# gkirgizov/die

Measured on AMD Instinct MI355X. Metric: env steps/sec on 4096^2 Physarum grid, higher is better.
Workload: dtype f32

## Files before the change

die_amd/csrc/die_pic.hip:

```cpp
#include "die_forward.h"
#include <stdlib.h>

typedef uint32_t pic_u4v __attribute__((ext_vector_type(4)));
typedef uint32_t pic_u2v __attribute__((ext_vector_type(2)));
template <typename T> struct Vec4;
template <> struct Vec4<float> {
    static __device__ __forceinline__ void ld(const float* p, float v[4]) {
        const uint4 t = *(const uint4*)p;
        v[0] = __uint_as_float(t.x); v[1] = __uint_as_float(t.y); v[2] = __uint_as_float(t.z); v[3] = __uint_as_float(t.w);
    }
    static __device__ __forceinline__ void st(float* p, const float v[4]) {
        *(uint4*)p = make_uint4(__float_as_uint(v[0]), __float_as_uint(v[1]), __float_as_uint(v[2]), __float_as_uint(v[3]));
    }
    static __device__ __forceinline__ void st_sel(bool nt, float* p, const float v[4]) {
        if (!nt) { st(p, v); return; }
        pic_u4v t; t.x = __float_as_uint(v[0]); t.y = __float_as_uint(v[1]); t.z = __float_as_uint(v[2]); t.w = __float_as_uint(v[3]);
        __builtin_nontemporal_store(t, (pic_u4v*)p);
    }
};
template <> struct Vec4<__half> {
    static __device__ __forceinline__ void ld(const __half* p, float v[4]) {
        const uint2 t = *(const uint2*)p;
        const __half2 a = *(const __half2*)&t.x, b = *(const __half2*)&t.y;
        v[0] = __low2float(a); v[1] = __high2float(a); v[2] = __low2float(b); v[3] = __high2float(b);
// ... 23 lines not shown
    uint32_t *off, *n, *s, *inc;
};

struct PicArgs {
    die_geo g;
    int ntx, nty, xs, ys;
    uint32_t xcd_wb_mul;
    int rp_c, rp_f;
    int margin;
    int fm_r, fm_c;
    uint32_t mg_c, mg_f;
    PicLayout in, out;
    float* dep;
    float *adx, *ady, *adep;
    const void* food;
    float rate_feed, w_dep, w_dist;
    int boundary, cost;
    long long* part_gain;
    uint32_t* error;
    uint4* rim;
    uint8_t* rim_code;
    uint32_t* rim_cnt;
    int rim_cap, rim_r;
    int sub_mode, sub_tx0, sub_ty0, sub_ntx, sub_nty;
    int halo_fresh;
    const float *ipgx, *ipgy;
    float *opgx, *opgy;
    const uint16_t* order;
    int order_len;
};
__device__ __forceinline__ void pic_xcd_tile(int& tx, int& ty, int ntx, uint32_t row0, uint32_t wb_mul, uint32_t nty) {
    const uint32_t wb = nty >> 3, banded = (wb << 3) * (uint32_t)ntx;
    const uint32_t L = (blockIdx.y - row0) * nty + blockIdx.x;
    if (wb == 0) return;
    if (L < banded) {
        const uint32_t k = L >> 3;
        tx = (int)(wb_mul ? __umulhi(k, wb_mul) : k / wb); ty = (int)((L & 7u) * wb + (k - (uint32_t)tx * wb));
    } else {
        const uint32_t r = L - banded, rem = nty - (wb << 3);
        tx = (int)(r / rem); ty = (int)((wb << 3) + (r - (uint32_t)tx * rem));
    }
}

#define PIC_ORDER_SPAN 512
__device__ __forceinline__ uint32_t pic_sload(const uint32_t* a) {
    uint32_t w;
// ... 85 lines not shown
    }
    template <int NB> __device__ __forceinline__ void issue(uint4 (&v)[NB]) const {
        int r0, cv, gy;
        where(r0, cv, gy);
#pragma unroll
        for (int q = 0; q < NB; ++q) v[q] = load(r0 + q * rp, gy);
    }
    template <int NB> __device__ __forceinline__ void commit(T* dst, const uint4 (&v)[NB]) const {
        int r0, cv, gy;
        where(r0, cv, gy);
        if (r0 >= rp) return;
        uint4* d = (uint4*)dst + (r0 * vpr + cv);
#pragma unroll
        for (int q = 0; q < NB; ++q) if (r0 + q * rp < rows) d[q * rp * vpr] = v[q];
        for (int row = r0 + NB * rp; row < rows; row += rp) ((uint4*)dst)[row * vpr + cv] = load(row, gy);
    }
};

#define PIC_RIM_CAP_MAX 224
#define PIC_LIST_CAP 512
static_assert(PIC_LIST_CAP >= PIC_K1_BLOCK, "the first round of candidates is one per thread");

#define PIC_AT(base, type, idx) (*(type*)((char*)(base) + (size_t)(uint32_t)((uint32_t)(idx) << 2)))
#define PIC_K1_MINW 6
#define PIC_K1_MINW_F16 8
template <typename T, int KIND, bool STAGE, bool ACT, bool RIM, bool TILED, bool MOM = false>
__global__ __launch_bounds__(PIC_K1_BLOCK, (sizeof(T) == 2 ? PIC_K1_MINW_F16 : PIC_K1_MINW)) void k_pic_forward_move(FwdArgs f, PicArgs p) {
    __builtin_amdgcn_s_setprio(3);
    f.pgx = MOM ? (float*)p.ipgx : nullptr; f.pgy = MOM ? (float*)p.ipgy : nullptr; f.step_base = nullptr; f.mask = nullptr;
    if (!MOM) { f.inertia = 0.f; f.noise_scale = 0.f; }
    f.normalized = 1;
    f.g = p.g;
    struct KArgs { FwdArgs f; PicArgs p; };
    static_assert(alignof(FwdArgs) == 8 && alignof(PicArgs) == 8 && sizeof(FwdArgs) % 8 == 0, "kernel-argument layout of k_pic_forward_move");
    const volatile KArgs __attribute__((address_space(4)))* ka = (const volatile KArgs __attribute__((address_space(4)))*)__builtin_amdgcn_kernarg_segment_ptr();
#define PIC_KP(field, type) ((type)ka->p.field)
    extern __shared__ __align__(16) unsigned char pic_smem[];
    __shared__ uint32_t s_base[9], s_pre[10];
    __shared__ unsigned long long s_cnt;
    __shared__ uint32_t s_next, s_nlist;
    __shared__ uint32_t s_inc[9];
    __shared__ __align__(4) uint8_t s_rimc[RIM ? PIC_RIM_CAP_MAX : 4];
    __shared__ uint32_t s_list[PIC_LIST_CAP];
    __shared__ long long s_gain[PIC_K1_BLOCK / DIE_WAVE];
    __shared__ uint32_t s_alv[TILED ? PIC_K1_BLOCK / DIE_WAVE : 1];
    const int NT = p.ntx * p.nty;
// ... 83 lines not shown
            }
            const unsigned long long m = __ballot(hit);
            uint32_t at = 0;
            if (lane == 0 && m) at = atomicAdd(&s_nlist, (uint32_t)__popcll(m));
            at = __shfl(at, 0, DIE_WAVE);
            if (hit) s_list[at + (uint32_t)__popcll(m & below)] = j;
        }
        PA_BARRIER();
        const uint32_t n_own = cb == 0 ? own : 0u, count = n_own + s_nlist;
        bool first = cb == 0;
        for (;;) {
            uint32_t c = 0;
            if (first) {
                c = (uint32_t)(wave * DIE_WAVE);
            } else {
                if (lane == 0) c = atomicAdd(&s_next, (uint32_t)DIE_WAVE);
                c = __shfl(c, 0, DIE_WAVE);
            }
            if (c >= count) break;
            const uint32_t idx = c + lane;
            const bool act = idx < count;
            bool stay = false;
            uint32_t X = 0, Y = 0, sid = 0, hh = 0, hl = 0;
            float af = 0.f, dep = 0.f;
            [[maybe_unused]] float pux = 0.f, puy = 0.f;
            double hd = 0.0;
            uint32_t code = 0;
            bool listed = false;
            if (act) {
                const uint32_t j = idx < n_own ? base0 + idx : s_list[idx - n_own];
                if (first && idx < n_own) {
                    X = pX; Y = pY; sid = pS; hh = pHh; hl = pHl; af = pA;
                } else {
                    const uint32_t *ix_ = PIC_KP(in.x, const uint32_t*), *iy_ = PIC_KP(in.y, const uint32_t*), *is_ = PIC_KP(in.slot, const uint32_t*);
                    const uint32_t *ihh_ = PIC_KP(in.hhi, const uint32_t*), *ihl_ = PIC_KP(in.hlo, const uint32_t*);
                    const float* ia_ = PIC_KP(in.agent_food, const float*);
                    X = PIC_AT(ix_, const uint32_t, j); Y = PIC_AT(iy_, const uint32_t, j); sid = PIC_AT(is_, const uint32_t, j);
                    hh = PIC_AT(ihh_, const uint32_t, j); hl = PIC_AT(ihl_, const uint32_t, j);
                    af = PIC_AT(ia_, const float, j);
                }
                hd = __hiloint2double((int)hh, (int)hl);
                const FwdOut o = STAGE ? die_forward_agent_mem<T, KIND, false, FwdTileMem<T, TILED>, true, false>(f, tm, X, Y, hd, sid, (int64_t)j)
                                       : die_forward_agent_mem<T, KIND, false, FwdGlobalMem<T, false>, true, false>(f, FwdGlobalMem<T, false>(f), X, Y, hd, sid, (int64_t)j);
                if (MOM) { pux = o.ux; puy = o.uy; }
                if (ACT && p.adx) { PIC_AT(p.adx, float, j) = o.dx; PIC_AT(p.ady, float, j) = o.dy; PIC_AT(p.adep, float, j) = o.dep; }
                if (p.boundary == DIE_BOUNDARY_WRAP) {
                    X += (uint32_t)die_q32_small(o.dx);
                    Y += (uint32_t)die_q32_small(o.dy);
                } else {
                    const int64_t qx = (int64_t)X + die_q32_small(o.dx), qy = (int64_t)Y + die_q32_small(o.dy);
                    X = (uint32_t)(qx < 0 ? 0 : (qx > 0xFFFFFFFFLL ? 0xFFFFFFFFLL : qx));
                    Y = (uint32_t)(qy < 0 ? 0 : (qy > 0xFFFFFFFFLL ? 0xFFFFFFFFLL : qy));
                }
                const int gcx = die_cell_u(X, p.g.gW), gcy = die_cell_u(Y, p.g.gH);
                const int cx = TILED ? die_plane_coord(gcx, p.g.ox, p.g.W, p.g.gW) : gcx;
                const int cy = TILED ? die_plane_coord(gcy, p.g.oy, p.g.H, p.g.gH) : gcy;
                const int ntx_ = cx >> p.xs, nty_ = cy >> p.ys;
                stay = ntx_ == tx && nty_ == ty;
                float fnew;
                if (STAGE) {
                    int rx = cx - x0, ry = cy - y0;
                    rx += rx < -FR ? p.g.W : 0; rx -= rx >= TX + FR ? p.g.W : 0;
                    ry += ry < -FC ? p.g.H : 0; ry -= ry >= TY + FC ? p.g.H : 0;
                    rx = min(max(rx + FR, 0), frows - 1);
                    if (ry >= -FC && ry < TY + FC) fnew = die_ld(s_food, (int64_t)(rx * fpitch + ry + FC));
                    else fnew = die_ld(food, (int64_t)cx * p.g.H + cy);
                } else {
                    fnew = die_ld(food, (int64_t)cx * p.g.H + cy);
                }
                const float consumed = p.rate_feed * fnew;
                const float cost = p.cost == DIE_COST_LINEAR ? p.w_dep * fabsf(o.dep) + p.w_dist * die_sqrt1(o.dx * o.dx + o.dy * o.dy) : 0.f;
                const float gained = consumed - cost;
                af += gained;
                if (!TILED || p.g.own_x1 == 0 || (cx >= p.g.own_x0 && cx < p.g.own_x1 && cy >= p.g.own_y0 && cy < p.g.own_y1)) { gsum += die_fix(gained); ++nowned; }
                hd = o.heading;
                dep = o.dep;
                int ddx = 0, ddy = 0;
                if (!stay) {
                    ddx = ntx_ - tx; ddy = nty_ - ty;
                    ddx = ddx > 1 ? ddx - p.ntx : (ddx < -1 ? ddx + p.ntx : ddx);
                    ddy = ddy > 1 ? ddy - p.nty : (ddy < -1 ? ddy + p.nty : ddy);
                    if (ddx < -1 || ddx > 1 || ddy < -1 || ddy > 1) { atomicOr(p.error, 2u); ddx = ddy = 0; }
                    else atomicAdd(&s_inc[(ddx + 1) * 3 + ddy + 1], 1u);
                }
                if (RIM) {
                    const int lx = cx & (TX - 1), ly = cy & (TY - 1), Rr = p.rim_r;
                    const int ex = lx < Rr ? 0 : (lx >= TX - Rr ? 2 : 1), ey = ly < Rr ? 0 : (ly >= TY - Rr ? 2 : 1);
                    code = (uint32_t)(((ddx + 1) * 3 + ddy + 1) * 9 + ex * 3 + ey);
                    listed = !stay || ex != 1 || ey != 1;
                }
            }
            const unsigned long long m_stay = __ballot(act && stay), m_leave = __ballot(act && !stay), m_rim = RIM ? __ballot(act && listed) : 0ull;
            unsigned long long base = 0;
            if (lane == 0) base = atomicAdd(&s_cnt, (unsigned long long)__popcll(m_stay) | ((unsigned long long)__popcll(m_leave) << 21) |
                                                    ((unsigned long long)__popcll(m_rim) << 42));
            base = __shfl(base, 0, DIE_WAVE);
            const uint32_t bf = (uint32_t)base & 0x1FFFFFu, bb = (uint32_t)(base >> 21) & 0x1FFFFFu, br = (uint32_t)(base >> 42) & 0x1FFFFFu;
            const uint32_t k = stay ? bf + (uint32_t)__popcll(m_stay & below) : on - 1u - (bb + (uint32_t)__popcll(m_leave & below));
            if (RIM && act && listed) {
                const uint32_t at = br + (uint32_t)__popcll(m_rim & below);
                if (at < (uint32_t)p.rim_cap) {
                    s_rimc[at] = (uint8_t)code;
                    PIC_KP(rim, uint4*)[(size_t)tile * p.rim_cap + at] = make_uint4(X, Y, sid, __float_as_uint(dep));
                }
            }
            if (act) {
                if (k < on) {
                    const uint32_t q = obase + k;
                    uint32_t *ox_ = PIC_KP(out.x, uint32_t*), *oy_ = PIC_KP(out.y, uint32_t*), *os_ = PIC_KP(out.slot, uint32_t*);
                    uint32_t *ohh_ = PIC_KP(out.hhi, uint32_t*), *ohl_ = PIC_KP(out.hlo, uint32_t*);
                    float *oa_ = PIC_KP(out.agent_food, float*), *od_ = PIC_KP(dep, float*);
                    PIC_AT(ox_, uint32_t, q) = X;
                    PIC_AT(oy_, uint32_t, q) = Y;
                    PIC_AT(oa_, float, q) = af;
                    PIC_AT(os_, uint32_t, q) = sid;
                    PIC_AT(ohh_, uint32_t, q) = (uint32_t)__double2hiint(hd);
                    PIC_AT(ohl_, uint32_t, q) = (uint32_t)__double2loint(hd);
                    PIC_AT(od_, float, q) = dep;
                    if (MOM && p.opgx) { PIC_AT(p.opgx, float, q) = pux; PIC_AT(p.opgy, float, q) = puy; }
                } else {
                    atomicOr(PIC_KP(error, uint32_t*), 1u);
                }
            }
            first = false;
        }
        if (cb + PIC_LIST_CAP < ncand) {
            PA_BARRIER();
            if (threadIdx.x == 0) { s_next = 0; s_nlist = 0; }
            PA_BARRIER();
        }
    }
    __builtin_amdgcn_s_setprio(3);
    gsum = die_wave_sum(gsum);
    if (lane == 0) s_gain[threadIdx.x / DIE_WAVE] = gsum;
    if (TILED) {
        const long long c = die_wave_sum((long long)nowned);
        if (lane == 0) s_alv[threadIdx.x / DIE_WAVE] = (uint32_t)c;
    }
    const int w_inc = nwaves > 1 ? 1 : 0, w_rim = nwaves > 2 ? 2 : 0;
    uint32_t* e_inc = nullptr; uint8_t* e_rimc = nullptr; uint32_t* e_rimn = nullptr; long long* e_gain = nullptr;
    if (wave == w_inc) e_inc = PIC_KP(out.inc, uint32_t*);
// ... 47 lines not shown
        const uint32_t j = first + i;
        uint32_t X = p.in.x[j], Y = p.in.y[j];
        const uint32_t sid = p.in.slot[j];
        const double hd = __hiloint2double((int)p.in.hhi[j], (int)p.in.hlo[j]);
        const FwdOut o = die_forward_agent_mem<T, KIND, false, FwdGlobalMem<T, false>, true>(f, mem, X, Y, hd, sid, (int64_t)j);
        if (p.adx) { p.adx[j] = o.dx; p.ady[j] = o.dy; p.adep[j] = o.dep; }
        if (p.boundary == DIE_BOUNDARY_WRAP) {
            X += (uint32_t)die_q32_small(o.dx);
            Y += (uint32_t)die_q32_small(o.dy);
        } else {
            const int64_t qx = (int64_t)X + die_q32_small(o.dx), qy = (int64_t)Y + die_q32_small(o.dy);
            X = (uint32_t)(qx < 0 ? 0 : (qx > 0xFFFFFFFFLL ? 0xFFFFFFFFLL : qx));
            Y = (uint32_t)(qy < 0 ? 0 : (qy > 0xFFFFFFFFLL ? 0xFFFFFFFFLL : qy));
        }
        const int cx = die_cell_u(X, p.g.gW), cy = die_cell_u(Y, p.g.gH);
        const uint32_t c = (uint32_t)cx * (uint32_t)p.g.H + (uint32_t)cy;
        const bool occupied = occ[c] != 0;
        const float consumed = occupied ? p.rate_feed * die_ld(food, (int64_t)c) : 0.f;
        const float cost = p.cost == DIE_COST_LINEAR ? p.w_dep * fabsf(o.dep) + p.w_dist * die_sqrt1(o.dx * o.dx + o.dy * o.dy) : 0.f;
        const float gained = consumed - cost;
        gsum += die_fix(gained);
        p.out.x[j] = X; p.out.y[j] = Y; p.out.agent_food[j] = p.in.agent_food[j] + gained; p.out.slot[j] = sid;
        p.out.hhi[j] = (uint32_t)__double2hiint(o.heading); p.out.hlo[j] = (uint32_t)__double2loint(o.heading);
        p.dep[j] = o.dep;
    }
    __shared__ long long s_g[DIE_BLOCK / DIE_WAVE];
    gsum = die_wave_sum(gsum);
    if ((threadIdx.x & (DIE_WAVE - 1)) == 0) s_g[threadIdx.x / DIE_WAVE] = gsum;
    __syncthreads();
    if (threadIdx.x == 0) {
        long long t = 0;
        for (int w = 0; w < DIE_BLOCK / DIE_WAVE; ++w) t += s_g[w];
        if (gridDim.x <= nslots) part[blockIdx.x] = t;
        else atomicAdd((unsigned long long*)&part[blockIdx.x % nslots], (unsigned long long)t);
    }
}

__device__ __forceinline__ void pic_turn_bits_fill(uint32_t* table, int64_t words, uint64_t seed, uint32_t step, int64_t first, int64_t stride) {
    for (int64_t b = first; b * 4 < words; b += stride) {
        const die_u32x4 r = die_philox((uint32_t)b, 0u, step, DIE_STREAM_TURN, (uint32_t)seed, (uint32_t)(seed >> 32));
        if (b * 4 + 3 < words) *(uint4*)(table + b * 4) = make_uint4(r.v[0], r.v[1], r.v[2], r.v[3]);
        else for (int q = 0; q < 4 && b * 4 + q < words; ++q) table[b * 4 + q] = r.v[q];
    }
}
__global__ __launch_bounds__(DIE_BLOCK) void k_turn_bits(uint32_t* table, int64_t words, uint64_t seed, uint32_t step) {
    pic_turn_bits_fill(table, words, seed, step, (int64_t)blockIdx.x * blockDim.x + threadIdx.x, (int64_t)gridDim.x * blockDim.x);
}
// ... 36 lines not shown
    if (FEED) {
        T* food = (T*)p.food;
#pragma unroll
        for (int q = 0; q < FG; ++q) {
            const int i = ((int)threadIdx.x + q * PIC_K2_BLOCK) * 4;
            if (i < TX * TY) { const int row = i / TY, col = i - row * TY; Vec4<T>::ld(food + (int64_t)(tx * TX + row) * p.g.H + ty * TY + col, fd[q]); }
        }
        (void)V;
    }
    for (int i = threadIdx.x; i < TX * TY / 2; i += PIC_K2_BLOCK) ((ulonglong2*)s_claim)[i] = make_ulonglong2(0ull, 0ull);
    pic_ranges_finish(mt, s_base, s_pre);
    const uint32_t total = s_pre[9], own = s_pre[1];
    for (uint32_t i0 = threadIdx.x; i0 < total; i0 += 2 * PIC_K2_BLOCK) {
        uint32_t X[2], Y[2], sid[2], db[2];
        bool has[2];
#pragma unroll
        for (int u = 0; u < 2; ++u) {
            const uint32_t idx = i0 + u * PIC_K2_BLOCK;
            has[u] = idx < total;
            if (has[u]) {
                int r = 0;
                while (idx >= s_pre[r + 1]) ++r;
                const uint32_t j = s_base[r] + (idx - s_pre[r]);
                X[u] = p.out.x[j]; Y[u] = p.out.y[j]; sid[u] = p.out.slot[j]; db[u] = __float_as_uint(p.dep[j]);
            }
        }
#pragma unroll
        for (int u = 0; u < 2; ++u) {
            if (!has[u]) continue;
            const uint32_t idx = i0 + u * PIC_K2_BLOCK;
            const int cx = die_cell((int64_t)X[u], p.g.gW), cy = die_cell((int64_t)Y[u], p.g.gH);
            if (idx >= own && ((cx >> XS) != tx || (cy >> YS) != ty)) continue;
            atomicMax(&s_claim[(cx & (TX - 1)) * TY + (cy & (TY - 1))], ((unsigned long long)(sid[u] + 1u) << 32) | (unsigned long long)db[u]);
        }
    }
    __syncthreads();
    static_assert(TY % 4 == 0, "16-byte stores");
#pragma unroll
    for (int g = 0; g < FG; ++g) {
        const int i = ((int)threadIdx.x + g * PIC_K2_BLOCK) * 4;
        if (i >= TX * TY) break;
        const int row = i / TY, col = i - row * TY;
        const ulonglong2 c01 = *(const ulonglong2*)&s_claim[i], c23 = *(const ulonglong2*)&s_claim[i + 2];
        const unsigned long long c[4] = {c01.x, c01.y, c23.x, c23.y};
        uint32_t o[4];
#pragma unroll
        for (int q = 0; q < 4; ++q) o[q] = c[q] ? (uint32_t)c[q] : DIE_DEP_EMPTY;
        const int64_t off = (int64_t)(tx * TX + row) * p.g.H + ty * TY + col;
        *(uint4*)(dep_plane + off) = make_uint4(o[0], o[1], o[2], o[3]);
        if (FEED && (c[0] | c[1] | c[2] | c[3])) {
            bool changed = false;
#pragma unroll
            for (int q = 0; q < 4; ++q) if (c[q] && fd[g][q] != 0.f) { fd[g][q] = fd[g][q] - p.rate_feed * fd[g][q]; changed = true; }
            if (changed) Vec4<T>::st((T*)p.food + off, fd[g]);
        }
    }
}

struct KbArgs {
    const void* chem;
    void* chem_next;
    const uint4* rim;
    const uint8_t* rim_code;
    const uint32_t* rim_cnt;
    int food_infinite;
    float keep;
    float w[2 * 4 + 1];
    die_step_result* result;
    long long alive_const;
    long long* status_out;
    const uint32_t* error;
    int nt_out;
    int n_part;
    uint32_t* turn_bits;
    int64_t turn_words;
    uint64_t turn_seed;
    uint32_t turn_step;
};

template <int XS, int YS> struct KbShape {
    static constexpr int BLOCK = ((1 << XS) * (1 << YS) >= 4096) ? 512 : 256;
    static constexpr int NE = 4;
    static constexpr int RIM_CAP = NE * BLOCK / 9 / 4 * 4;
    static_assert(RIM_CAP <= PIC_RIM_CAP_MAX, "the agent kernel's list holds it");
};

#define PIC_KB_MINW 8
template <typename T, int XS, int YS, int R, bool TILED>
__global__ __launch_bounds__((KbShape<XS, YS>::BLOCK), PIC_KB_MINW) void k_pic_resolve_diffuse(PicArgs p, KbArgs a) {
    constexpr int TX = 1 << XS, TY = 1 << YS, BLOCK = KbShape<XS, YS>::BLOCK;
    constexpr int A = 16 / (int)sizeof(T);
    constexpr int WR = TX + 2 * R, WC = TY + 2 * R;
    constexpr int CP = TY + 2 * A, NV = CP / A;
    static_assert(R >= 1 && R <= 4 && R <= A, "the rim lies inside one vector beside the tile");
    extern __shared__ __align__(16) unsigned char kb_smem[];
    float* s_chem = (float*)kb_smem;
    uint32_t* s_claim = (uint32_t*)(s_chem + WR * CP);
    float* s_tmp = (float*)s_claim;
    __shared__ uint32_t s_off[9], s_n[9], s_rn[9];
    __shared__ uint32_t s_own[2];
    __shared__ unsigned char s_lut[9 * 81 + 3];
    constexpr int CAPR = KbShape<XS, YS>::RIM_CAP, NE = KbShape<XS, YS>::NE;
    const int NT = p.ntx * p.nty;
    const uint32_t row0 = p.sub_mode == 1 ? 0u : 1u;
    if (row0 && blockIdx.y == 0) {
        if (blockIdx.x == 0) {
            uint32_t* s_sum = (uint32_t*)kb_smem;
            const int per = (NT + BLOCK - 1) / BLOCK;
            const int lo = threadIdx.x * per, hi = min(lo + per, NT);
            uint32_t sum = 0;
            for (int t = lo; t < hi; ++t) sum += p.out.s[t] + p.out.inc[t];
            s_sum[threadIdx.x] = sum;
            __syncthreads();
            for (int o = 1; o < BLOCK; o <<= 1) {
                const uint32_t v = (int)threadIdx.x >= o ? s_sum[threadIdx.x - o] : 0u;
                __syncthreads();
                s_sum[threadIdx.x] += v;
// ... 96 lines not shown
        const int sx = e / 3 - 1, sy = e % 3 - 1;
        const bool here = (ux == 0 || ux == -sx) && (uy == 0 || uy == -sy) && !(q == 0 && dd == 4);
        s_lut[t] = here ? (unsigned char)((ux + 1) * 3 + uy + 1) : (unsigned char)0xFF;
    }
    __syncthreads();
    auto window_commit = [&](int q, const uint4 u) {
        const int i = (int)threadIdx.x + q * BLOCK;
        if (i >= WR * NV) return;
        const int r = i / NV, v = i - r * NV;
        float* dst = s_chem + r * CP + v * A;
        if constexpr (sizeof(T) == 4) {
            *(uint4*)dst = u;
        } else {
            auto lo = [](uint32_t w) { return __half2float(__ushort_as_half((unsigned short)(w & 0xFFFFu))); };
            auto hi = [](uint32_t w) { return __half2float(__ushort_as_half((unsigned short)(w >> 16))); };
            *(float4*)dst = make_float4(lo(u.x), hi(u.x), lo(u.y), hi(u.y));
            *(float4*)(dst + 4) = make_float4(lo(u.z), hi(u.z), lo(u.w), hi(u.w));
        }
    };
    window_commit(0, cv0);
    if constexpr (NCV > 1) window_commit(1, cv1);
    if constexpr (NCV > 2) window_commit(2, cv2);
    const uint32_t own0 = s_own[0], nown = s_own[1];
    auto window_cell = [&](uint32_t X, uint32_t Y, int ux, int uy) {
        const int cx = pic_row<TILED>(p.g, X), cy = pic_col<TILED>(p.g, Y);
        const int r = ux * TX + (cx & (TX - 1)) + R, c = uy * TY + (cy & (TY - 1)) + R;
        return (r >= 0 && r < WR && c >= 0 && c < WC) ? (uint32_t)(r * WC + c) | ((uint32_t)r << 16) : 0xFFFFFFFFu;
    };
    static_assert(WR * WC < (1 << 16) && WR < (1 << 15), "window cell and row in one word");
    auto rim_decode = [&](int m, uint32_t& uc) {
        uc = 0xFFu;
        if (rl >= 9 || (uint32_t)(ri + m) >= s_rn[rl] || s_rn[rl] > (uint32_t)CAPR) return 0xFFFFFFFFu;
        const uint32_t code = (rcodes >> (8 * m)) & 255u;
        if (code >= 81u) return 0xFFFFFFFFu;
        uc = s_lut[rl * 81 + code];
        return uc == 0xFFu ? 0xFFFFFFFFu : (uint32_t)(ri + m);
    };
#define PIC_KB_U 4
    auto scan_segment = [&](int l, bool apply) {
        const uint32_t lo = l == 0 ? own0 + nown : s_off[l], hi = s_off[l] + s_n[l];
        for (uint32_t j0 = lo + threadIdx.x; j0 < hi; j0 += PIC_KB_U * BLOCK) {
            uint32_t X[PIC_KB_U], Y[PIC_KB_U], S[PIC_KB_U], D[PIC_KB_U];
#pragma unroll
            for (int u = 0; u < PIC_KB_U; ++u) {
                const uint32_t j = j0 + (uint32_t)u * BLOCK;
                X[u] = Y[u] = S[u] = D[u] = 0u;
                if (j < hi) { X[u] = p.out.x[j]; Y[u] = p.out.y[j]; S[u] = p.out.slot[j]; if (apply) D[u] = __float_as_uint(p.dep[j]); }
            }
#pragma unroll
            for (int u = 0; u < PIC_KB_U; ++u) {
                if (j0 + (uint32_t)u * BLOCK >= hi) continue;
                const int cx = pic_row<TILED>(p.g, X[u]), cy = pic_col<TILED>(p.g, Y[u]);
                int rr = cx - x0, rc = cy - y0;
                rr = rr > W / 2 ? rr - W : (rr < -(W / 2) ? rr + W : rr);
                rc = rc > H / 2 ? rc - H : (rc < -(H / 2) ? rc + H : rc);
                if (rr < -R || rr >= TX + R || rc < -R || rc >= TY + R) continue;
                const uint32_t widx = (uint32_t)((rr + R) * WC + rc + R), s1 = S[u] + 1u;
                if (!apply) atomicMax(&s_claim[widx], s1);
                else if (s_claim[widx] == s1) {
                    float* c = &s_chem[(rr + R) * CP + rc + A];
                    *c = die_as_stored<T>(*c + __uint_as_float(D[u]));
                }
            }
        }
    };
    uint32_t over = 0;
#pragma unroll
    for (int l = 0; l < 9; ++l) over |= s_rn[l] > (uint32_t)CAPR ? 1u << l : 0u;
    constexpr int FG = (TX * TY / 4 + BLOCK - 1) / BLOCK;
    float fd[FG][4];
    uint32_t cw[2 + NE], cs[2 + NE], cd[2 + NE];
    {
        uint32_t X[2 + NE], Y[2 + NE], uc[NE];
        const uint32_t rj[NE] = {rim_decode(0, uc[0]), rim_decode(1, uc[1]), rim_decode(2, uc[2]), rim_decode(3, uc[3])};
        const uint4* rrec = a.rim + (size_t)ring_tile(rl < 9 ? rl : 0) * CAPR;
#pragma unroll
        for (int u = 0; u < 2 + NE; ++u) {
            cw[u] = 0xFFFFFFFFu; cs[u] = 0u; cd[u] = 0u; X[u] = Y[u] = 0u;
            if (u < 2) {
                if (threadIdx.x + u * BLOCK < nown) {
                    const uint32_t j = own0 + threadIdx.x + u * BLOCK;
                    X[u] = p.out.x[j]; Y[u] = p.out.y[j]; cs[u] = p.out.slot[j] + 1u; cd[u] = __float_as_uint(p.dep[j]); cw[u] = 0u;
                }
            } else if (rj[u - 2] != 0xFFFFFFFFu) {
                const uint4 q = rrec[rj[u - 2]];
                X[u] = q.x; Y[u] = q.y; cs[u] = q.z + 1u; cd[u] = q.w; cw[u] = 0u;
            }
        }
        if (!a.food_infinite) {
#pragma unroll
            for (int q = 0; q < FG; ++q) {
                const int i = ((int)threadIdx.x + q * BLOCK) * 4;
                if (i < TX * TY) { const int row = i / TY, col = i - row * TY; Vec4<T>::ld(food + (int64_t)(x0 + row) * H + y0 + col, fd[q]); }
            }
        }
#pragma unroll
        for (int u = 0; u < 2 + NE; ++u) {
            if (cw[u] == 0xFFFFFFFFu) continue;
            cw[u] = u < 2 ? window_cell(X[u], Y[u], 0, 0) : window_cell(X[u], Y[u], (int)uc[u - 2] / 3 - 1, (int)uc[u - 2] % 3 - 1);
            if (cw[u] != 0xFFFFFFFFu) atomicMax(&s_claim[cw[u] & 0xFFFFu], cs[u]);
        }
    }
    for (uint32_t i0 = threadIdx.x + 2 * BLOCK; i0 < nown; i0 += PIC_KB_U * BLOCK) {
        uint32_t X[PIC_KB_U], Y[PIC_KB_U], S[PIC_KB_U];
#pragma unroll
        for (int u = 0; u < PIC_KB_U; ++u) {
            const uint32_t i = i0 + (uint32_t)u * BLOCK, j = own0 + i;
            X[u] = Y[u] = S[u] = 0u;
            if (i < nown) { X[u] = p.out.x[j]; Y[u] = p.out.y[j]; S[u] = p.out.slot[j]; }
        }
#pragma unroll
        for (int u = 0; u < PIC_KB_U; ++u) {
            if (i0 + (uint32_t)u * BLOCK >= nown) continue;
            const uint32_t w_ = window_cell(X[u], Y[u], 0, 0);
            if (w_ != 0xFFFFFFFFu) atomicMax(&s_claim[w_ & 0xFFFFu], S[u] + 1u);
        }
    }
    if (over) for (int l = 0; l < 9; ++l) if (over >> l & 1u) scan_segment(l, false);
    __syncthreads();
    auto deposit = [&](uint32_t widx, uint32_t s1, uint32_t db) {
        if (widx == 0xFFFFFFFFu || s_claim[widx & 0xFFFFu] != s1) return;
        const uint32_t r = widx >> 16, c = (widx & 0xFFFFu) - r * WC;
        float* q = &s_chem[r * CP + c - R + A];
        *q = die_as_stored<T>(*q + __uint_as_float(db));
    };
#pragma unroll
    for (int u = 0; u < 2 + NE; ++u) deposit(cw[u], cs[u], cd[u]);
    for (uint32_t i0 = threadIdx.x + 2 * BLOCK; i0 < nown; i0 += PIC_KB_U * BLOCK) {
        uint32_t X[PIC_KB_U], Y[PIC_KB_U], S[PIC_KB_U], D[PIC_KB_U];
#pragma unroll
        for (int u = 0; u < PIC_KB_U; ++u) {
            const uint32_t i = i0 + (uint32_t)u * BLOCK, j = own0 + i;
            X[u] = Y[u] = S[u] = D[u] = 0u;
            if (i < nown) { X[u] = p.out.x[j]; Y[u] = p.out.y[j]; S[u] = p.out.slot[j]; D[u] = __float_as_uint(p.dep[j]); }
        }
#pragma unroll
        for (int u = 0; u < PIC_KB_U; ++u)
            if (i0 + (uint32_t)u * BLOCK < nown) deposit(window_cell(X[u], Y[u], 0, 0), S[u] + 1u, D[u]);
    }
    if (over) for (int l = 0; l < 9; ++l) if (over >> l & 1u) scan_segment(l, true);
    if (!a.food_infinite) {
#pragma unroll
        for (int g = 0; g < FG; ++g) {
            const int i = ((int)threadIdx.x + g * BLOCK) * 4;
            if (i >= TX * TY) break;
            const int row = i / TY, col = i - row * TY;
            const uint32_t* c = &s_claim[(row + R) * WC + col + R];
            const bool occ[4] = {c[0] != 0u && fd[g][0] != 0.f, c[1] != 0u && fd[g][1] != 0.f, c[2] != 0u && fd[g][2] != 0.f, c[3] != 0u && fd[g][3] != 0.f};
            if (occ[0] || occ[1] || occ[2] || occ[3]) {
#pragma unroll
                for (int q = 0; q < 4; ++q) if (occ[q]) fd[g][q] = fd[g][q] - p.rate_feed * fd[g][q];
                Vec4<T>::st_sel(a.nt_out != 0, food + (int64_t)(x0 + row) * H + y0 + col, fd[g]);
            }
        }
    }
    __syncthreads();
    constexpr int RB = TX >= 64 ? 16 : 8;
    for (int item = threadIdx.x; item < WC * (TX / RB); item += BLOCK) {
        const int rb = item / WC, c = item - rb * WC;
        const float* src = s_chem + (rb * RB) * CP + c - R + A;
        float win[2 * R + 1];
#pragma unroll
        for (int k = 0; k < 2 * R; ++k) win[k + 1] = src[k * CP];
#pragma unroll
// ... 429 lines not shown
        DIE_REQUIRE(ok && vpr_c <= 64 && vpr_f <= 64, "die_pic_forward_env_step: staged rows of %d / %d vectors", vpr_c, vpr_f);
    }
    DIE_REQUIRE(!stage || (m->W < (1 << 23) && m->H < (1 << 23) && (int64_t)m->W * m->H < (1ll << 31)),
                "die_pic_forward_env_step: plane too large for the 24-bit index arithmetic of the staging loop");
    DIE_REQUIRE(!stage || m->H % V == 0, "die_pic_forward_env_step: plane rows must be whole 16-byte vectors");
    const size_t lds = stage ? ((size_t)(TX + 2 * P) * (TY + 2 * P) + (size_t)(TX + 2 * k.fm_r) * (TY + 2 * k.fm_c)) * esz : 0;
    const int stages = p->stages ? p->stages : 7;
    const int R = (int)(4.0 * (double)d->diffuse_sigma + 0.5);
    const bool two = p->rim != nullptr && p->rim_code != nullptr && p->rim_cnt != nullptr &&
                     pic_two_launch_rule(worldmax, p->tile_xs, p->tile_ys, step_scale, d->diffuse_sigma, d->diffuse_mode);
    if (!two) DIE_REQUIRE(p->dep_plane, "die_pic_forward_env_step: this step needs the three-launch form: dep_plane is null");
    DIE_REQUIRE(two || !p->sub_mode, "die_pic_forward_env_step: subsets of the tiles exist in the two-launch form only");
    DIE_REQUIRE(!(dead && p->sub_mode), "die_pic_forward_env_step: subsets of the tiles and dead slots do not combine");
    if (tiled && !(two && stage)) {
        die_set_error("die_pic_forward_env_step: a decomposed world's tile runs the two-launch form with staged tiles only (probe reach %d, radius %d)", P, R);
        return DIE_ERR_UNSUPPORTED;
    }
    if (tiled && ((m->gW != m->W && m->gW - m->W < 2 * k.margin + 2) || (m->gH != m->H && m->gH - m->H < 2 * k.margin + 2))) {
        die_set_error("die_pic_forward_env_step: the planes (%d x %d) nearly span the world (%d x %d): the taps around an agent are mapped "
                      "from its own cell (FwdTileMem::home), which needs %d cells of world beyond the planes", m->W, m->H, m->gW, m->gH, 2 * k.margin + 2);
        return DIE_ERR_UNSUPPORTED;
    }
    k.rim = (uint4*)p->rim; k.rim_code = p->rim_code; k.rim_cnt = p->rim_cnt; k.rim_cap = (int)die_pic_rim_cap(p->tile_xs, p->tile_ys); k.rim_r = R;
    const bool feed_in_k2 = !d->food_infinite;
    int block = p->k1_threads > 0 ? p->k1_threads : (TX * TY >= 4096 ? 512 : 256);
    DIE_REQUIRE(block % DIE_WAVE == 0 && block >= DIE_WAVE && block <= PIC_K1_BLOCK, "die_pic_forward_env_step: k1_threads %d", block);
    k.rp_c = stage ? block / vpr_c : 1; k.rp_f = stage ? block / vpr_f : 1;
    const bool physarum = g->kind == DIE_AGENT_PHYSARUM;
    const int64_t turn_words = (p->turn_slots + 127) / 128 * 4;
    if (physarum) {
        DIE_REQUIRE(p->turn_bits && p->turn_slots > 0, "die_pic_forward_env_step: turn_bits / turn_slots (a table over every slot id) missing");
        f.turn_bits = p->turn_bits;
        if ((stages & 1) && (!p->turn_ready || !two) && !g->turn_sign) {
            const int64_t blocks = (turn_words / 4 + DIE_BLOCK - 1) / DIE_BLOCK;
            k_turn_bits<<<(int)(blocks < 1024 ? blocks : 1024), DIE_BLOCK, 0, s>>>(p->turn_bits, turn_words, g->seed, g->step);
        }
    }
    if (p->order && two && !tiled && !p->sub_mode && (k.nty & 7) == 0 && NT <= 65536) {
        k.order = p->order; k.order_len = NT >> 3;
        if ((stages & 1) && (!p->order_ready || (g->step % PIC_ORDER_PERIOD) == 0))
            k_pic_order<<<dim3(8, ((NT >> 3) + PIC_ORDER_SPAN - 1) / PIC_ORDER_SPAN), PIC_ORDER_BLOCK, 0, s>>>(k.in.n, k.ntx, k.nty, p->order);
    }
    if (stages & 1) {
#define DIE_PIC_K1(T, STAGE, LDS) do { if (two) launch_forward_move<T, STAGE, true>(g->kind, f, k, NT, block, LDS, s, mom); \
                                       else launch_forward_move<T, STAGE, false>(g->kind, f, k, NT, block, LDS, s, mom); } while (0)
        if (tiled) {
// ... 86 lines not shown
    die_gradient_agent gg = *g;
    for (int32_t i = 0; i < n_steps; ++i) {
        const int rc = die_pic_forward_env_step(&mm, &pp, (from + i) & 1, &gg, nullptr, d, results + i, stream);
        if (rc != DIE_OK) return rc;
        g_pic_run_done = i + 1;
        void* t = mm.chem; mm.chem = mm.chem_next; mm.chem_next = t;
        gg.step += 1u;
        pp.turn_ready = 1;
        pp.order_ready = 1;
    }
    return DIE_OK;
}

__global__ __launch_bounds__(DIE_BLOCK) void k_pic_action_physarum(int64_t N, const uint32_t* hhi, const uint32_t* hlo, const float* dep,
                                                                  float scale, float* dx, float* dy, float* adep) {
    const int64_t stride = (int64_t)gridDim.x * blockDim.x;
    for (int64_t n = (int64_t)blockIdx.x * blockDim.x + threadIdx.x; n < N; n += stride) {
        float ux, uy;
        die_polar2xy_heading(__hiloint2double((int)hhi[n], (int)hlo[n]), 1.f, &ux, &uy);
        ux += 0.f;
        uy += 0.f;
        dx[n] = ux * scale;
        dy[n] = uy * scale;
        adep[n] = dep[n];
    }
}

extern "C" int die_pic_action_physarum(const die_pic* p, int32_t lay, const die_gradient_agent* g, const die_action* act, void* stream) {
    DIE_REQUIRE(p && g && act && (lay == 0 || lay == 1), "die_pic_action_physarum: null argument");
    DIE_REQUIRE(g->kind == DIE_AGENT_PHYSARUM && g->normalized_grad && g->inertia == 0.f && g->noise_scale == 0.f,
                "die_pic_action_physarum: a normalised PhysarumAgent without inertia or noise");
    const die_pic_layout& L = p->layout[lay];
    DIE_REQUIRE(p->N > 0 && act->N == p->N, "die_pic_action_physarum: the action holds %lld entries, the layout %lld", (long long)act->N, (long long)p->N);
    DIE_REQUIRE(L.heading_hi && L.heading_lo && p->dep && act->dx && act->dy && act->deposit, "die_pic_action_physarum: null array");
    int64_t grid = (p->N + DIE_BLOCK - 1) / DIE_BLOCK;
    k_pic_action_physarum<<<(int)(grid < 8192 ? grid : 8192), DIE_BLOCK, 0, (hipStream_t)stream>>>(
        p->N, L.heading_hi, L.heading_lo, p->dep, g->scale, act->dx, act->dy, act->deposit);
    DIE_CHECK_LAUNCH("die_pic_action_physarum");
    return DIE_OK;
}

extern "C" int die_agents_mark_owner(const die_medium* m, const die_agents* a, void* stream) {
    DIE_REQUIRE(m && a && m->owner && a->x && a->y && a->alive && a->N > 0, "die_agents_mark_owner: null argument");
    DIE_REQUIRE(m->epoch >= 1 && m->epoch <= DIE_OWNER_EPOCH_MAX, "die_agents_mark_owner: bad epoch %d", m->epoch);
    int64_t g = (a->N + DIE_BLOCK - 1) / DIE_BLOCK;
    k_mark_owner<<<(int)(g < 8192 ? g : 8192), DIE_BLOCK, 0, (hipStream_t)stream>>>(die_geo_of(m), a->N, m->epoch, a->x, a->y, a->slot,
                                                                                    a->alive, (unsigned long long*)m->owner);
// ... 4 lines not shown
```

die_amd/pic.py:

```python
import ctypes as C
import os
import weakref
from typing import Optional, Tuple

import numpy as np
import torch

from . import _lib
from .device_array import _ptr, stream_ptr

TILE_SHAPES = ((6, 6), (5, 6), (4, 5))


def pick_tile(W: int, H: int, reach_cells: float, shapes=TILE_SHAPES) -> Optional[Tuple[int, int]]:
    for xs, ys in shapes:
        TX, TY = 1 << xs, 1 << ys
        if W % TX == 0 and H % TY == 0 and W // TX >= 3 and H // TY >= 3 and reach_cells <= min(TX, TY) - 1:
            return xs, ys
    return None


def step_scale(agent) -> float:
    key = (agent._scale, agent._inertia, agent._noise_scale)
    hit = agent.__dict__.get('_pic_step_scale')
# ... 1 lines not shown
        return hit[1]
    import numpy as np
    bound = _lib.lib.die_pic_step_bound(float(agent._inertia), float(agent._noise_scale))
    value = float(np.float32(agent._scale) * np.float32(bound))
    agent.__dict__['_pic_step_scale'] = (key, value)
    return value


def lazy_ok(agent) -> bool:
    return agent._kind == _lib.DIE_AGENT_PHYSARUM and agent._turn_sign is None


class PicState:

    def __init__(self, env, tile: Tuple[int, int]):
        self.xs, self.ys = tile
        W, H = env.medium.W, env.medium.H
        self.NT = int(_lib.lib.die_pic_tiles(W, H, self.xs, self.ys))
        if self.NT <= 0:
            raise ValueError(f'tile shape 2^{tile} is not available')
        dev, N = env.device, int(env.agents.x.numel())
        self.cap = N
        self.meta = [torch.zeros((4, self.NT), dtype=torch.int32, device=dev) for _ in range(2)]
        self.dep = torch.empty(N, dtype=torch.float32, device=dev)
        self.fused = bool(getattr(env, '_pic_fused', True))
        cap = int(_lib.lib.die_pic_rim_cap(self.xs, self.ys))
        self.rim = torch.zeros((self.NT * cap, 4), dtype=torch.int32, device=dev) if self.fused else None
        self.rim_code = torch.zeros(self.NT * cap, dtype=torch.uint8, device=dev) if self.fused else None
        self.rim_cnt = torch.zeros(self.NT, dtype=torch.int32, device=dev) if self.fused else None
        self._plane_shape = (W, H)
        self._world_shape = (env.medium.world[0], env.medium.world[1]) if env.medium.world is not None else (W, H)
        self._n_agents = int(env.agents.N)
        self._dep_plane = None if self.fused else torch.empty((W, H), dtype=torch.float32, device=dev)
        self.turn_slots = max(N, int(getattr(env, 'world_agents', 0) or 0))
        self.turn_bits = torch.zeros(4 * ((self.turn_slots + 127) // 128), dtype=torch.int32, device=dev)
        self._turn_for = None
        nty = H >> self.ys
        self.order = torch.zeros(self.NT, dtype=torch.int16, device=dev) \
            if (self.fused and env.medium.world is None and nty % 8 == 0 and self.NT <= 65536 and os.environ.get('DIE_PIC_ORDER', '1') != '0') else None
        self._order_ready = False
        self.n_alive = int(getattr(env, '_pic_n_alive', 0) or 0)
        self.occ = torch.zeros(W * H, dtype=torch.uint8, device=dev) if 0 < self.n_alive < N else None
        self.part = torch.zeros(2 * self.NT, dtype=torch.int64, device=dev)
        self.error = torch.zeros(1, dtype=torch.int32, device=dev)
        i32 = lambda: torch.empty(N, dtype=torch.int32, device=dev)
        self.spare = [i32(), i32(), torch.empty(N, dtype=torch.float32, device=dev), i32(), i32()]
        self.spare_pg = None
# ... 224 lines not shown
```

Before: 7499.

## Carry sensed food with each agent and feed only claimed cells in K2

K1 now saves the food value it read at each agent's cell next to the deposit (the dep buffer becomes float pairs). In the untiled case, rim records hold the flat cell index and that food value in place of X/Y. K2 then updates food only at cells whose claim an agent wins, so the full-tile food read-modify-write pass is skipped. This trades a dense food sweep for scattered per-agent stores plus wider dep traffic. Correctness depends on each cell having at most one winning agent and on the cell index fitting in 32 bits.

```diff
diff --git a/die_amd/csrc/die_pic.hip b/die_amd/csrc/die_pic.hip
--- a/die_amd/csrc/die_pic.hip
+++ b/die_amd/csrc/die_pic.hip
@@ -69,6 +69,7 @@
     uint8_t* rim_code;
     uint32_t* rim_cnt;
     int rim_cap, rim_r;
+    int h_shift;
     int sub_mode, sub_tx0, sub_ty0, sub_ntx, sub_nty;
     int halo_fresh;
     const float *ipgx, *ipgy;
@@ -200,6 +201,8 @@
 static_assert(PIC_LIST_CAP >= PIC_K1_BLOCK, "the first round of candidates is one per thread");
 
 #define PIC_AT(base, type, idx) (*(type*)((char*)(base) + (size_t)(uint32_t)((uint32_t)(idx) << 2)))
+#define PIC_PAIR(base, idx) (*(float2*)((char*)(base) + ((size_t)(uint32_t)((uint32_t)(idx) << 2) << 1)))
+#define PIC_DEP(base, idx) ((base)[2 * (size_t)(idx)])
 #define PIC_K1_MINW 6
 #define PIC_K1_MINW_F16 8
 template <typename T, int KIND, bool STAGE, bool ACT, bool RIM, bool TILED, bool MOM = false>
@@ -329,7 +332,8 @@
             const bool act = idx < count;
             bool stay = false;
             uint32_t X = 0, Y = 0, sid = 0, hh = 0, hl = 0;
-            float af = 0.f, dep = 0.f;
+            float af = 0.f, dep = 0.f, fund = 0.f;
+            uint32_t cell = 0;
             [[maybe_unused]] float pux = 0.f, puy = 0.f;
             double hd = 0.0;
             uint32_t code = 0;
@@ -375,6 +379,8 @@
                 } else {
                     fnew = die_ld(food, (int64_t)cx * p.g.H + cy);
                 }
+                fund = fnew;
+                if (RIM && !TILED) cell = (uint32_t)cx * (uint32_t)p.g.H + (uint32_t)cy;
                 const float consumed = p.rate_feed * fnew;
                 const float cost = p.cost == DIE_COST_LINEAR ? p.w_dep * fabsf(o.dep) + p.w_dist * die_sqrt1(o.dx * o.dx + o.dy * o.dy) : 0.f;
                 const float gained = consumed - cost;
@@ -408,7 +414,8 @@
                 const uint32_t at = br + (uint32_t)__popcll(m_rim & below);
                 if (at < (uint32_t)p.rim_cap) {
                     s_rimc[at] = (uint8_t)code;
-                    PIC_KP(rim, uint4*)[(size_t)tile * p.rim_cap + at] = make_uint4(X, Y, sid, __float_as_uint(dep));
+                    PIC_KP(rim, uint4*)[(size_t)tile * p.rim_cap + at] = TILED ? make_uint4(X, Y, sid, __float_as_uint(dep))
+                                                                               : make_uint4(cell, __float_as_uint(fund), sid, __float_as_uint(dep));
                 }
             }
             if (act) {
@@ -423,7 +430,7 @@
                     PIC_AT(os_, uint32_t, q) = sid;
                     PIC_AT(ohh_, uint32_t, q) = (uint32_t)__double2hiint(hd);
                     PIC_AT(ohl_, uint32_t, q) = (uint32_t)__double2loint(hd);
-                    PIC_AT(od_, float, q) = dep;
+                    PIC_PAIR(od_, q) = make_float2(dep, fund);
                     if (MOM && p.opgx) { PIC_AT(p.opgx, float, q) = pux; PIC_AT(p.opgy, float, q) = puy; }
                 } else {
                     atomicOr(PIC_KP(error, uint32_t*), 1u);
@@ -517,7 +524,7 @@
         gsum += die_fix(gained);
         p.out.x[j] = X; p.out.y[j] = Y; p.out.agent_food[j] = p.in.agent_food[j] + gained; p.out.slot[j] = sid;
         p.out.hhi[j] = (uint32_t)__double2hiint(o.heading); p.out.hlo[j] = (uint32_t)__double2loint(o.heading);
-        p.dep[j] = o.dep;
+        PIC_DEP(p.dep, j) = o.dep;
     }
     __shared__ long long s_g[DIE_BLOCK / DIE_WAVE];
     gsum = die_wave_sum(gsum);
@@ -600,7 +607,7 @@
                 int r = 0;
                 while (idx >= s_pre[r + 1]) ++r;
                 const uint32_t j = s_base[r] + (idx - s_pre[r]);
-                X[u] = p.out.x[j]; Y[u] = p.out.y[j]; sid[u] = p.out.slot[j]; db[u] = __float_as_uint(p.dep[j]);
+                X[u] = p.out.x[j]; Y[u] = p.out.y[j]; sid[u] = p.out.slot[j]; db[u] = __float_as_uint(PIC_DEP(p.dep, j));
             }
         }
 #pragma unroll
@@ -633,6 +640,14 @@
             if (changed) Vec4<T>::st((T*)p.food + off, fd[g]);
         }
     }
+}
+
+__device__ __forceinline__ void pic_food_store(bool nt, float* p, float v) {
+    if (nt) __builtin_nontemporal_store(v, p); else *p = v;
+}
+__device__ __forceinline__ void pic_food_store(bool nt, __half* p, float v) {
+    const unsigned short h = __half_as_ushort(die_f2h(v));
+    if (nt) __builtin_nontemporal_store(h, (unsigned short*)p); else *(unsigned short*)p = h;
 }
 
 struct KbArgs {
@@ -671,6 +686,7 @@
     constexpr int WR = TX + 2 * R, WC = TY + 2 * R;
     constexpr int CP = TY + 2 * A, NV = CP / A;
     static_assert(R >= 1 && R <= 4 && R <= A, "the rim lies inside one vector beside the tile");
+    constexpr bool HAND = !TILED;
     extern __shared__ __align__(16) unsigned char kb_smem[];
     float* s_chem = (float*)kb_smem;
     uint32_t* s_claim = (uint32_t*)(s_chem + WR * CP);
@@ -813,10 +829,20 @@
     if constexpr (NCV > 1) window_commit(1, cv1);
     if constexpr (NCV > 2) window_commit(2, cv2);
     const uint32_t own0 = s_own[0], nown = s_own[1];
-    auto window_cell = [&](uint32_t X, uint32_t Y, int ux, int uy) {
-        const int cx = pic_row<TILED>(p.g, X), cy = pic_col<TILED>(p.g, Y);
+    auto window_cell_of = [&](int cx, int cy, int ux, int uy) {
         const int r = ux * TX + (cx & (TX - 1)) + R, c = uy * TY + (cy & (TY - 1)) + R;
         return (r >= 0 && r < WR && c >= 0 && c < WC) ? (uint32_t)(r * WC + c) | ((uint32_t)r << 16) : 0xFFFFFFFFu;
+    };
+    auto window_cell = [&](uint32_t X, uint32_t Y, int ux, int uy) { return window_cell_of(pic_row<TILED>(p.g, X), pic_col<TILED>(p.g, Y), ux, uy); };
+    auto window_cell_rec = [&](uint32_t cell, int ux, int uy) {
+        const uint32_t cx = p.h_shift >= 0 ? cell >> p.h_shift : cell / (uint32_t)H;
+        return window_cell_of((int)cx, (int)(cell - cx * (uint32_t)H), ux, uy);
+    };
+    auto feed_cell = [&](uint32_t r, uint32_t c, uint32_t fb) {
+        const uint32_t tr = r - (uint32_t)R, tc = c - (uint32_t)R;
+        const float fo = __uint_as_float(fb);
+        if (a.food_infinite || tr >= (uint32_t)TX || tc >= (uint32_t)TY || !(fo != 0.f)) return;
+        pic_food_store(a.nt_out != 0, food + ((int64_t)(x0 + (int)tr) * H + y0 + (int)tc), fo - p.rate_feed * fo);
     };
     static_assert(WR * WC < (1 << 16) && WR < (1 << 15), "window cell and row in one word");
     auto rim_decode = [&](int m, uint32_t& uc) {
@@ -831,12 +857,15 @@
     auto scan_segment = [&](int l, bool apply) {
         const uint32_t lo = l == 0 ? own0 + nown : s_off[l], hi = s_off[l] + s_n[l];
         for (uint32_t j0 = lo + threadIdx.x; j0 < hi; j0 += PIC_KB_U * BLOCK) {
-            uint32_t X[PIC_KB_U], Y[PIC_KB_U], S[PIC_KB_U], D[PIC_KB_U];
+            uint32_t X[PIC_KB_U], Y[PIC_KB_U], S[PIC_KB_U], D[PIC_KB_U], F[PIC_KB_U];
 #pragma unroll
             for (int u = 0; u < PIC_KB_U; ++u) {
                 const uint32_t j = j0 + (uint32_t)u * BLOCK;
-                X[u] = Y[u] = S[u] = D[u] = 0u;
-                if (j < hi) { X[u] = p.out.x[j]; Y[u] = p.out.y[j]; S[u] = p.out.slot[j]; if (apply) D[u] = __float_as_uint(p.dep[j]); }
+                X[u] = Y[u] = S[u] = D[u] = F[u] = 0u;
+                if (j < hi) {
+                    X[u] = p.out.x[j]; Y[u] = p.out.y[j]; S[u] = p.out.slot[j];
+                    if (apply) { const float2 df = PIC_PAIR(p.dep, j); D[u] = __float_as_uint(df.x); F[u] = __float_as_uint(df.y); }
+                }
             }
 #pragma unroll
             for (int u = 0; u < PIC_KB_U; ++u) {
@@ -851,6 +880,7 @@
                 else if (s_claim[widx] == s1) {
                     float* c = &s_chem[(rr + R) * CP + rc + A];
                     *c = die_as_stored<T>(*c + __uint_as_float(D[u]));
+                    if (HAND) feed_cell((uint32_t)(rr + R), (uint32_t)(rc + R), F[u]);
                 }
             }
         }
@@ -859,26 +889,28 @@
 #pragma unroll
     for (int l = 0; l < 9; ++l) over |= s_rn[l] > (uint32_t)CAPR ? 1u << l : 0u;
     constexpr int FG = (TX * TY / 4 + BLOCK - 1) / BLOCK;
-    float fd[FG][4];
-    uint32_t cw[2 + NE], cs[2 + NE], cd[2 + NE];
+    [[maybe_unused]] float fd[FG][4];
+    uint32_t cw[2 + NE], cs[2 + NE], cd[2 + NE], cf[2 + NE];
     {
         uint32_t X[2 + NE], Y[2 + NE], uc[NE];
         const uint32_t rj[NE] = {rim_decode(0, uc[0]), rim_decode(1, uc[1]), rim_decode(2, uc[2]), rim_decode(3, uc[3])};
         const uint4* rrec = a.rim + (size_t)ring_tile(rl < 9 ? rl : 0) * CAPR;
 #pragma unroll
         for (int u = 0; u < 2 + NE; ++u) {
-            cw[u] = 0xFFFFFFFFu; cs[u] = 0u; cd[u] = 0u; X[u] = Y[u] = 0u;
+            cw[u] = 0xFFFFFFFFu; cs[u] = 0u; cd[u] = 0u; cf[u] = 0u; X[u] = Y[u] = 0u;
             if (u < 2) {
                 if (threadIdx.x + u * BLOCK < nown) {
                     const uint32_t j = own0 + threadIdx.x + u * BLOCK;
-                    X[u] = p.out.x[j]; Y[u] = p.out.y[j]; cs[u] = p.out.slot[j] + 1u; cd[u] = __float_as_uint(p.dep[j]); cw[u] = 0u;
+                    const float2 df = PIC_PAIR(p.dep, j);
+                    X[u] = p.out.x[j]; Y[u] = p.out.y[j]; cs[u] = p.out.slot[j] + 1u; cd[u] = __float_as_uint(df.x); cf[u] = __float_as_uint(df.y); cw[u] = 0u;
                 }
             } else if (rj[u - 2] != 0xFFFFFFFFu) {
                 const uint4 q = rrec[rj[u - 2]];
                 X[u] = q.x; Y[u] = q.y; cs[u] = q.z + 1u; cd[u] = q.w; cw[u] = 0u;
-            }
-        }
-        if (!a.food_infinite) {
+                if (HAND) cf[u] = q.y;
+            }
+        }
+        if (!HAND && !a.food_infinite) {
 #pragma unroll
             for (int q = 0; q < FG; ++q) {
                 const int i = ((int)threadIdx.x + q * BLOCK) * 4;
@@ -888,7 +920,9 @@
 #pragma unroll
         for (int u = 0; u < 2 + NE; ++u) {
             if (cw[u] == 0xFFFFFFFFu) continue;
-            cw[u] = u < 2 ? window_cell(X[u], Y[u], 0, 0) : window_cell(X[u], Y[u], (int)uc[u - 2] / 3 - 1, (int)uc[u - 2] % 3 - 1);
+            if (u < 2) cw[u] = window_cell(X[u], Y[u], 0, 0);
+            else if (HAND) cw[u] = window_cell_rec(X[u], (int)uc[u - 2] / 3 - 1, (int)uc[u - 2] % 3 - 1);
+            else cw[u] = window_cell(X[u], Y[u], (int)uc[u - 2] / 3 - 1, (int)uc[u - 2] % 3 - 1);
             if (cw[u] != 0xFFFFFFFFu) atomicMax(&s_claim[cw[u] & 0xFFFFu], cs[u]);
         }
     }
@@ -909,28 +943,32 @@
     }
     if (over) for (int l = 0; l < 9; ++l) if (over >> l & 1u) scan_segment(l, false);
     __syncthreads();
-    auto deposit = [&](uint32_t widx, uint32_t s1, uint32_t db) {
+    auto deposit = [&](uint32_t widx, uint32_t s1, uint32_t db, uint32_t fb) {
         if (widx == 0xFFFFFFFFu || s_claim[widx & 0xFFFFu] != s1) return;
         const uint32_t r = widx >> 16, c = (widx & 0xFFFFu) - r * WC;
         float* q = &s_chem[r * CP + c - R + A];
         *q = die_as_stored<T>(*q + __uint_as_float(db));
+        if (HAND) feed_cell(r, c, fb);
     };
 #pragma unroll
-    for (int u = 0; u < 2 + NE; ++u) deposit(cw[u], cs[u], cd[u]);
+    for (int u = 0; u < 2 + NE; ++u) deposit(cw[u], cs[u], cd[u], cf[u]);
     for (uint32_t i0 = threadIdx.x + 2 * BLOCK; i0 < nown; i0 += PIC_KB_U * BLOCK) {
-        uint32_t X[PIC_KB_U], Y[PIC_KB_U], S[PIC_KB_U], D[PIC_KB_U];
+        uint32_t X[PIC_KB_U], Y[PIC_KB_U], S[PIC_KB_U], D[PIC_KB_U], F[PIC_KB_U];
 #pragma unroll
         for (int u = 0; u < PIC_KB_U; ++u) {
             const uint32_t i = i0 + (uint32_t)u * BLOCK, j = own0 + i;
-            X[u] = Y[u] = S[u] = D[u] = 0u;
-            if (i < nown) { X[u] = p.out.x[j]; Y[u] = p.out.y[j]; S[u] = p.out.slot[j]; D[u] = __float_as_uint(p.dep[j]); }
+            X[u] = Y[u] = S[u] = D[u] = F[u] = 0u;
+            if (i < nown) {
+                const float2 df = PIC_PAIR(p.dep, j);
+                X[u] = p.out.x[j]; Y[u] = p.out.y[j]; S[u] = p.out.slot[j]; D[u] = __float_as_uint(df.x); F[u] = __float_as_uint(df.y);
+            }
         }
 #pragma unroll
         for (int u = 0; u < PIC_KB_U; ++u)
-            if (i0 + (uint32_t)u * BLOCK < nown) deposit(window_cell(X[u], Y[u], 0, 0), S[u] + 1u, D[u]);
+            if (i0 + (uint32_t)u * BLOCK < nown) deposit(window_cell(X[u], Y[u], 0, 0), S[u] + 1u, D[u], F[u]);
     }
     if (over) for (int l = 0; l < 9; ++l) if (over >> l & 1u) scan_segment(l, true);
-    if (!a.food_infinite) {
+    if (!HAND && !a.food_infinite) {
 #pragma unroll
         for (int g = 0; g < FG; ++g) {
             const int i = ((int)threadIdx.x + g * BLOCK) * 4;
@@ -1406,6 +1444,9 @@
         return DIE_ERR_UNSUPPORTED;
     }
     k.rim = (uint4*)p->rim; k.rim_code = p->rim_code; k.rim_cnt = p->rim_cnt; k.rim_cap = (int)die_pic_rim_cap(p->tile_xs, p->tile_ys); k.rim_r = R;
+    DIE_REQUIRE(!two || tiled || (int64_t)m->W * m->H < ((int64_t)1 << 32), "die_pic_forward_env_step: %d x %d cells do not fit a rim record's 32-bit cell index", m->W, m->H);
+    k.h_shift = -1;
+    for (int q = 0; q < 31; ++q) if (m->H == (1 << q)) k.h_shift = q;
     const bool feed_in_k2 = !d->food_infinite;
     int block = p->k1_threads > 0 ? p->k1_threads : (TX * TY >= 4096 ? 512 : 256);
     DIE_REQUIRE(block % DIE_WAVE == 0 && block >= DIE_WAVE && block <= PIC_K1_BLOCK, "die_pic_forward_env_step: k1_threads %d", block);
@@ -1538,7 +1579,7 @@
         uy += 0.f;
         dx[n] = ux * scale;
         dy[n] = uy * scale;
-        adep[n] = dep[n];
+        adep[n] = PIC_DEP(dep, n);
     }
 }
 
diff --git a/die_amd/pic.py b/die_amd/pic.py
--- a/die_amd/pic.py
+++ b/die_amd/pic.py
@@ -47,7 +47,7 @@
         dev, N = env.device, int(env.agents.x.numel())
         self.cap = N
         self.meta = [torch.zeros((4, self.NT), dtype=torch.int32, device=dev) for _ in range(2)]
-        self.dep = torch.empty(N, dtype=torch.float32, device=dev)
+        self.dep = torch.empty((N, 2), dtype=torch.float32, device=dev)
         self.fused = bool(getattr(env, '_pic_fused', True))
         cap = int(_lib.lib.die_pic_rim_cap(self.xs, self.ys))
         self.rim = torch.zeros((self.NT * cap, 4), dtype=torch.int32, device=dev) if self.fused else None
```

Result: slower. 7371 (-1.7%).
